# bernardo-torres/1d-spectral-optimal-transport

Hardware: AMD Instinct MI355X
Metric: sot_loss_evals_per_sec (higher is better)
Workload: dtype f32

## Files before the change

1d-spectral-optimal-transport_amd/csrc/sot_forward_full.inc:

```

#ifdef SOT_STAMPS
#define SOT_PH(sacc, i) do { if ((sacc) != nullptr) { __builtin_amdgcn_sched_barrier(0); const unsigned long long now_ = __builtin_readcyclecounter(); \
                              (sacc)[i] += now_ - (sacc)[15]; (sacc)[15] = now_; __builtin_amdgcn_sched_barrier(0); } } while (0)
#else
#define SOT_PH(sacc, i) do { } while (0)
#endif

template <int NSTEPS>
__device__ __forceinline__ float mass_column_nx(const float* part, int c)
{
    constexpr int NFULL = NSTEPS >> 4;
    constexpr int NREAD = NFULL + ((NSTEPS & 15) ? 1 : 0);
    float pre[NREAD];
#pragma unroll
    for (int h = 0; h < NREAD; ++h) pre[h] = part[(h << 5) + c];
    float a0 = 0.0f, a1 = 0.0f, a2 = 0.0f, a3 = 0.0f;
#pragma unroll
    for (int h = 0; h < NFULL; ++h) {
        a0 = pre[h];
        a1 += a0; a0 = 0.0f;
        if ((((h + 1) << 4) & (15 << 4)) == 0) {
            a2 += a1; a1 = 0.0f;
            if ((((h + 1) << 4) & (15 << 8)) == 0) { a3 += a2; a2 = 0.0f; }
        }
// ... 401 lines not shown
#pragma unroll
            for (int s2 = 0; s2 < CHUNK; ++s2) acc += v[s2];
            part[id] = acc;
        }
    }
    }
    SOT_PH(sacc, 3);
    if constexpr (!COLUMNS) row_sync<NW>();
    SOT_PH(sacc, 4);
    __builtin_amdgcn_s_setprio(kMassPrio);
    if (NW >= 2) {
        if (wv < 2 && !(wv == 1 && dn)) {
            const float* raw = wv ? V : U;
            float* cb = colbuf + 32 * wv;
            if (lane < 32) {
                if constexpr (RT) cb[lane] = mass_column<SQ>(raw, part + wv * NT, mp, lane);
                else cb[lane] = mass_column_nx<Geo::NSTEPS>(part + wv * NT, lane);
            }
            __builtin_amdgcn_fence(__ATOMIC_RELEASE, "wavefront");
            __builtin_amdgcn_wave_barrier();
            __builtin_amdgcn_fence(__ATOMIC_ACQUIRE, "wavefront");
            float S;
            if constexpr (RT) S = mass_fold<SQ>(raw, cb, mp.n);
            else S = mass_fold_nx<(SQ && !PRESQ), N, SWZ>(raw, cb);
            if (lane == 0) { Sv[wv] = S; Sv[2 + wv] = 1.0f / guard_mass(S); }
        }
    } else {
        const int half = lane >> 5, col = lane & 31;
        const bool use_y = half && !dn;
        float* cb = colbuf + 32 * half;
        if constexpr (RT) cb[col] = mass_column<SQ>(use_y ? V : U, part + (use_y ? NT : 0), mp, col);
        else cb[col] = mass_column_nx<Geo::NSTEPS>(part + (use_y ? NT : 0), col);
        __builtin_amdgcn_fence(__ATOMIC_RELEASE, "wavefront");
        __builtin_amdgcn_wave_barrier();
        __builtin_amdgcn_fence(__ATOMIC_ACQUIRE, "wavefront");
        float S;
        if constexpr (RT) S = mass_fold<SQ>(use_y ? V : U, cb, mp.n);
        else S = mass_fold_nx<(SQ && !PRESQ), N, SWZ>(use_y ? V : U, cb);
        if (col == 0) { Sv[half] = S; Sv[2 + half] = 1.0f / guard_mass(S); }
    }
    __builtin_amdgcn_s_setprio(0);
    const int e0 = t * CPT;
    const int h0 = e0 + 4 * ownf, h1 = e0 + 4 * (1 - ownf);
    if (x_ident) {
        if constexpr (CPT == 8) {
            const float4 v0 = *reinterpret_cast<const float4*>(U + h0), v1 = *reinterpret_cast<const float4*>(U + h1);
            wx[0] = v0.x; wx[1] = v0.y; wx[2] = v0.z; wx[3] = v0.w; wx[4] = v1.x; wx[5] = v1.y; wx[6] = v1.z; wx[7] = v1.w;
        } else {
#pragma unroll
            for (int k = 0; k < CPT; ++k) wx[k] = U[e0 + k];
        }
    } else if (psx != nullptr) {
#pragma unroll
        for (int k = 0; k < CPT; ++k) wx[k] = U[psx[k]];
    } else {
#pragma unroll
        for (int k = 0; k < CPT; ++k) {
            const int sx = (e0 + k < (RT ? a.n : N)) ? a.xperm[e0 + k] : N + 1;
            wx[k] = U[SWZ ? (sx ^ (((sx >> 5) & 1) << 2)) : sx];
        }
    }
    if (y_ident) {
        if constexpr (CPT == 8) {
            const float4 v0 = *reinterpret_cast<const float4*>(V + h0), v1 = *reinterpret_cast<const float4*>(V + h1);
            wy[0] = v0.x; wy[1] = v0.y; wy[2] = v0.z; wy[3] = v0.w; wy[4] = v1.x; wy[5] = v1.y; wy[6] = v1.z; wy[7] = v1.w;
        } else {
#pragma unroll
            for (int k = 0; k < CPT; ++k) wy[k] = V[e0 + k];
        }
    } else if (psy != nullptr) {
#pragma unroll
        for (int k = 0; k < CPT; ++k) wy[k] = V[psy[k]];
    } else {
#pragma unroll
        for (int k = 0; k < CPT; ++k) {
            const int sy = (e0 + k < (RT ? a.n : N)) ? a.yperm[e0 + k] : N + 1;
            wy[k] = V[SWZ ? (sy ^ (((sy >> 5) & 1) << 2)) : sy];
        }
    }
    if ((N < Geo::CAP || RT) && e0 + CPT > (RT ? a.n : N)) {
#pragma unroll
        for (int k = 0; k < CPT; ++k) {
            if (e0 + k >= (RT ? a.n : N)) { wx[k] = 0.0f; wy[k] = 0.0f; }
        }
    }
    SOT_PH(sacc, 5);
    row_sync<NW>();
    SOT_PH(sacc, 6);

    Sx = Sv[0]; Sy = dn ? Sx : Sv[1];
    const float rSx = Sv[2], rSy = dn ? rSx : Sv[3];
    const float Sxh = guard_mass(Sx), Syh = guard_mass(Sy);
    double px[CPT], py[CPT];
    double runx = 0.0, runy = 0.0;
    {
        float qx[CPT], qy[CPT];
        uint32_t risk = 0xFFFFFFFFu;
#pragma unroll
        for (int k = 0; k < CPT; ++k) {
            qx[k] = div_by_row_constant((SQ && !PRESQ) ? wx[k] * wx[k] : wx[k], Sxh, rSx, risk);
            qy[k] = div_by_row_constant((SQ && !PRESQ) ? wy[k] * wy[k] : wy[k], Syh, rSy, risk);
        }
        const bool slow = (risk < kFastDivMinBits) || !(Sxh <= 0x1p40f) || !(Syh <= 0x1p40f);
        if (__builtin_amdgcn_ballot_w64(slow) != 0ull) {
            asm volatile("; IEEE division fallback" ::: "memory");
#pragma unroll
            for (int k = 0; k < CPT; ++k) {
                qx[k] = ((SQ && !PRESQ) ? wx[k] * wx[k] : wx[k]) / Sxh;
                qy[k] = ((SQ && !PRESQ) ? wy[k] * wy[k] : wy[k]) / Syh;
            }
        }
#pragma unroll
        for (int k = 0; k < CPT; ++k) {
            runx += (double)qx[k]; runy += (double)qy[k];
            px[k] = runx; py[k] = runy;
        }
    }
    const double inx = wave_incl_scan(runx), iny = wave_incl_scan(runy);
    double exx = wave_shift_right1(inx), exy = wave_shift_right1(iny);
    if (NW > 1 && lane == kWave - 1) { wtot[wv] = inx; wtot[NW + wv] = iny; }
    SOT_PH(sacc, 7);
    row_sync<NW>();
    SOT_PH(sacc, 8);
    if constexpr (NW > 1) {
        double ox = 0.0, oy = 0.0;
        for (int w = 0; w < wv; ++w) { ox += wtot[w]; oy += wtot[NW + w]; }
        exx += ox; exy += oy;
    }
#pragma unroll
    for (int k = 0; k < CPT; ++k) { cu[k] = (float)(exx + px[k]); cv[k] = (float)(exy + py[k]); }
    if constexpr (TO_LDS) {
        if (CPT % 4 == 0 && (N == Geo::CAP || e0 + CPT <= N)) {
#pragma unroll
            for (int k = 0; k + 3 < CPT; k += 4) {
                *reinterpret_cast<float4*>(U + e0 + k) = make_float4(cu[k], cu[k + 1], cu[k + 2], cu[k + 3]);
                *reinterpret_cast<float4*>(V + e0 + k) = make_float4(cv[k], cv[k + 1], cv[k + 2], cv[k + 3]);
            }
        } else {
#pragma unroll
            for (int k = 0; k < CPT; ++k) {
                if (e0 + k < N) { U[e0 + k] = cu[k]; V[e0 + k] = cv[k]; }
            }
        }
    }
    if (nxt_x != nullptr) fetch_row<G, CPT, NX>(nxt_x, nxt_y, t, a.n, rx, ry);
    if constexpr (TO_LDS) row_sync<NW>();
}

template <int G, int CPT, int ROWS, int NX>
__device__ __forceinline__ void owner_perm_slots(const FwdArgs& a, const int* perm, int t, int (&ps)[CPT])
{
    using Geo = FullGeo<G, CPT, ROWS, false, NX>;
    constexpr int N = Geo::N;
    const int nreal = Geo::RT ? a.n : N;
#pragma unroll
    for (int k = 0; k < CPT; ++k) {
        const int sx = (t * CPT + k < nreal) ? perm[t * CPT + k] : N + 1;
        ps[k] = Geo::SWZ ? (sx ^ (((sx >> 5) & 1) << 2)) : sx;
    }
}

constexpr int kFwdMinWaves = 1;
constexpr int kRt512MinWaves = 4;

template <int G, int CPT, int ROWS, int GRAD, int NX>
__device__ __forceinline__ void rowpos_row_setup(const FwdArgs& a, const FullCtx& c, int64_t rowc, int (&ix)[CPT], int (&iy)[CPT], int (&psx)[CPT], int (&psy)[CPT])
{
    using Geo = FullGeo<G, CPT, ROWS, GRAD, NX>;
    constexpr int N = Geo::N, NW = Geo::NW, PAD = Geo::PAD;
    static_assert(ROWS == 1 && NX == 0 && CPT == 8, "per-row positions: one row per workgroup, rows that fill the 8-element geometry");
    const int t = c.t;
    const uint16_t* const pr = a.perm_in + rowc * (2 * (int64_t)N);
    const float* const xp = a.xpos + rowc * a.xps;
    const float* const yp = a.ypos + rowc * a.yps;
    const uint4 qx = *reinterpret_cast<const uint4*>(pr + t * CPT), qy = *reinterpret_cast<const uint4*>(pr + N + t * CPT);
    float vx[CPT], vy[CPT];
#pragma unroll
    for (int k = 0; k < CPT; ++k) { vx[k] = xp[t + k * G]; vy[k] = yp[t + k * G]; }
    const uint32_t wqx[4] = {qx.x, qx.y, qx.z, qx.w}, wqy[4] = {qy.x, qy.y, qy.z, qy.w};
#pragma unroll
    for (int k = 0; k < CPT; ++k) {
        ix[k] = (int)((wqx[k >> 1] >> (16 * (k & 1))) & (uint32_t)(N - 1));
        iy[k] = (int)((wqy[k >> 1] >> (16 * (k & 1))) & (uint32_t)(N - 1));
        psx[k] = Geo::SWZ ? (ix[k] ^ (((ix[k] >> 5) & 1) << 2)) : ix[k];
        psy[k] = Geo::SWZ ? (iy[k] ^ (((iy[k] >> 5) & 1) << 2)) : iy[k];
    }
    float* const Um = c.U; float* const Vm = c.V;
#pragma unroll
    for (int k = 0; k < CPT; ++k) { Um[t + k * G] = vx[k]; Vm[t + k * G] = vy[k]; }
    row_sync<NW>();
    float gx[CPT], gy[CPT];
#pragma unroll
    for (int k = 0; k < CPT; ++k) { gx[k] = Um[ix[k]]; gy[k] = Vm[iy[k]]; }
    float* const PXw = const_cast<float*>(c.PX); float* const PYw = const_cast<float*>(c.PY);
    *reinterpret_cast<float4*>(PXw + t * CPT) = make_float4(gx[0], gx[1], gx[2], gx[3]);
    *reinterpret_cast<float4*>(PXw + t * CPT + 4) = make_float4(gx[4], gx[5], gx[6], gx[7]);
    *reinterpret_cast<float4*>(PYw + t * CPT) = make_float4(gy[0], gy[1], gy[2], gy[3]);
    *reinterpret_cast<float4*>(PYw + t * CPT + 4) = make_float4(gy[4], gy[5], gy[6], gy[7]);
    if (t < PAD) PXw[t - PAD] = gx[0];
    if (t == G - 1) { PXw[N] = gx[CPT - 1]; PYw[N] = gy[CPT - 1]; }
    row_sync<NW>();
}

template <int G, int CPT, int ROWS, int PM, bool LIM, bool SQ, int NX = 0, bool RP = false>
__global__ __launch_bounds__(ROWS * G, (G == 512 && NX < 0) ? kRt512MinWaves : (CPT == 17) ? kFwd17MinWaves : kFwdMinWaves) void sot_forward_full_kernel(const FwdArgs a)
{
    static_assert(!RP || (ROWS == 1 && NX == 0 && CPT == 8), "per-row positions: one row per workgroup, rows that fill the 8-element geometry");
    using Geo = FullGeo<G, CPT, ROWS, false, NX>;
    constexpr FullLayout L = Geo::L;
    constexpr int N = Geo::N, NW = Geo::NW, E = Geo::E, GA = Geo::GA, PAD = Geo::PAD;
    extern __shared__ __attribute__((aligned(16))) float smem[];
    const int64_t row_step = (int64_t)gridDim.x * ROWS;
    int64_t row0 = (int64_t)blockIdx.x * ROWS;
    float rx[CPT], ry[CPT];
    FullCtx cm = full_setup<G, CPT, ROWS, false, NX, RP>(a, smem);
    if constexpr (RP) { cm.x_ident = false; cm.y_ident = false; }
    const FullCtx c = cm;
    if constexpr (NW == 1) __syncthreads();
    const int rg = c.rg, t = c.t, lane = c.lane, wv = c.wv;
    float* const V = c.V; float* const red = c.red;
    const float* const Uw = c.Uw;
    if (row0 < a.B) {
        const int64_t r = min(row0 + rg, a.B - 1);
        fetch_row<G, CPT, NX>(a.x + r * a.xs, a.y + r * a.ys, t, a.n, rx, ry);
    }

#ifdef SOT_STAMPS
    unsigned long long sbuf[16] = {};
    unsigned long long* const sacc = (threadIdx.x == 0 && blockIdx.x == gridDim.x / 2) ? sbuf : nullptr;
#else
    constexpr unsigned long long* sacc = nullptr;
#endif
    constexpr bool HOIST_PERM = CPT <= 9;
    int psx[HOIST_PERM ? CPT : 1] = {}, psy[HOIST_PERM ? CPT : 1] = {};
    if constexpr (HOIST_PERM && !RP) {
        if (!c.x_ident) owner_perm_slots<G, CPT, ROWS, NX>(a, a.xperm, t, psx);
        if (!c.y_ident) owner_perm_slots<G, CPT, ROWS, NX>(a, a.yperm, t, psy);
    }
    for (; row0 < a.B; row0 += row_step) {
        const int64_t row = row0 + rg;
        const bool valid = row < a.B;
        const bool more = row0 + row_step < a.B;
        const int64_t rn = min(row0 + row_step + rg, a.B - 1);
        float wx[CPT], wy[CPT], cu[CPT], cv[CPT];
        float Sx, Sy;
#ifdef SOT_STAMPS
        if (sacc != nullptr) sacc[15] = __builtin_readcyclecounter();
#endif
        if constexpr (RP) {
            int ix[CPT], iy[CPT];
            rowpos_row_setup<G, CPT, ROWS, false, NX>(a, c, min(row, a.B - 1), ix, iy, psx, psy);
        }
        full_build_cdfs<G, CPT, ROWS, false, SQ, NX>(a, c, rx, ry, more ? a.x + rn * a.xs : nullptr,
                                                     more ? a.y + rn * a.ys : nullptr, wx, wy, Sx, Sy, cu, cv, sacc, HOIST_PERM ? psx : nullptr,
                                                     HOIST_PERM ? psy : nullptr);
        SOT_PH(sacc, 9);

        float acc = 0.0f;
        __builtin_amdgcn_s_setprio(kWalkPrio);
        if (GA == G || t < GA) {
            constexpr int VOFF = L.nU - L.padcap + PAD;
            const int D0 = t * E;
            (void)VOFF;
            const uint32_t ub1 = lds_addr(Uw) - 4u;
            const uint32_t vd1 = lds_addr(V) + 4u * (uint32_t)D0 + ub1;
            const uint32_t pb = merge_path_fixed32<N + PAD, N>(ub1, vd1, D0);
            SOT_PH(sacc, 10);
            const uint32_t ou = pb + 4u;
            const uint32_t ov = vd1 - pb;
            constexpr uint32_t ROWB = 4u * (uint32_t)L.rowf;
            if (ROWS == 1 || rg == ROWS - 1) acc = merge_walk_full<E, PM, LIM, ROWB>(ou, ov, D0 == 0, a.p);
            else if (ROWS == 2 || rg == ROWS - 2) acc = merge_walk_full<E, PM, LIM, 2u * ROWB>(ou, ov, D0 == 0, a.p);
            else if (ROWS == 3 || rg == ROWS - 3) acc = merge_walk_full<E, PM, LIM, 3u * ROWB>(ou, ov, D0 == 0, a.p);
            else acc = merge_walk_full<E, PM, LIM, 4u * ROWB>(ou, ov, D0 == 0, a.p);
        }
        __builtin_amdgcn_s_setprio(0);
        SOT_PH(sacc, 11);
        acc = wave_sum(acc);
        if (NW == 1) {
            if (lane == 0 && valid && a.row_loss) store_row_loss(a.row_loss, row, acc, a.mt.counters != nullptr);
            row_sync<NW>();
        } else {
            if (lane == 0) red[wv] = acc;
            row_sync<NW>();
            if (t == 0 && valid && a.row_loss) {
                float tot = red[0];
#pragma unroll
                for (int w = 1; w < NW; ++w) tot += red[w];
                store_row_loss(a.row_loss, row, tot, a.mt.counters != nullptr);
            }
        }
        SOT_PH(sacc, 12);
#ifdef SOT_STAMPS
        if (sacc != nullptr) sacc[0] += 1;
#endif
    }
#ifdef SOT_STAMPS
    if (sacc != nullptr) { for (int i = 0; i < 16; ++i) g_stamps[i] = sacc[i]; }
#endif
    if (a.mt.counters != nullptr) batch_mean_tail<ROWS * G>(a.mt, a.row_loss, a.B, reinterpret_cast<double*>(smem));
}


constexpr int kAreaMinWaves = 1;
template <int G, int CPT, int ROWS, bool SQ, int NX = 0>
__global__ __launch_bounds__(ROWS * G, (CPT == 17) ? kFwd17MinWaves : kAreaMinWaves) void sot_area_full_kernel(const FwdArgs a)
{
    using Geo = FullGeo<G, CPT, ROWS, false, NX>;
    constexpr FullLayout L = Geo::L;
    constexpr int N = Geo::N, NW = Geo::NW;
    extern __shared__ __attribute__((aligned(16))) float smem[];
    const int64_t row_step = (int64_t)gridDim.x * ROWS;
    int64_t row0 = (int64_t)blockIdx.x * ROWS;
    const int tid = threadIdx.x;
    FullCtx c;
    c.rg = __builtin_amdgcn_readfirstlane(tid / G);
    c.t = tid - c.rg * G;
    c.lane = tid & (kWave - 1);
    c.wv = __builtin_amdgcn_readfirstlane(c.t >> 6);
    const int rg = c.rg, t = c.t, lane = c.lane, wv = c.wv;
    float rx[CPT], ry[CPT];
    if (row0 < a.B) {
        const int64_t r = min(row0 + rg, a.B - 1);
        fetch_row<G, CPT, NX>(a.x + r * a.xs, a.y + r * a.ys, t, a.n, rx, ry);
    }
    c.dn = a.flags & SOT_FLAG_DONT_NORMALIZE;
    float* const base = smem + rg * L.rowf;
    c.U = base + L.padcap; c.V = base + L.nU; c.part = base + L.part; c.colbuf = base + L.colbuf;
    c.wtot = reinterpret_cast<double*>(base + L.wtot);
    c.red = base + L.red; c.Sv = c.red + NW;
    c.Uw = c.U; c.PX = nullptr; c.PY = nullptr;
    c.x_ident = true; c.y_ident = true;
    if (a.ident != nullptr) { c.x_ident = a.ident[0] != 0; c.y_ident = a.ident[1] != 0; }
    float dx[CPT];
    {
        const int e0 = t * CPT;
        float pe[CPT + 1];
        const int nreal = Geo::RT ? a.n : N;
#pragma unroll
        for (int k = 0; k <= CPT; ++k) pe[k] = a.xpos[min(e0 + k, nreal - 1)];
#pragma unroll
        for (int k = 0; k < CPT; ++k) dx[k] = (e0 + k + 1 < nreal) ? pe[k + 1] - pe[k] : 0.0f;
    }
    float* const red = c.red;
#ifdef SOT_STAMPS
    unsigned long long sbuf[16] = {};
    unsigned long long* const sacc = (threadIdx.x == 0 && blockIdx.x == gridDim.x / 2) ? sbuf : nullptr;
#endif

    for (; row0 < a.B; row0 += row_step) {
        const int64_t row = row0 + rg;
        const bool valid = row < a.B;
        const bool more = row0 + row_step < a.B;
        const int64_t rn = min(row0 + row_step + rg, a.B - 1);
        float wx[CPT], wy[CPT], cu[CPT], cv[CPT];
        float Sx, Sy;
#ifdef SOT_STAMPS
        if (sacc != nullptr) sacc[15] = __builtin_readcyclecounter();
        full_build_cdfs<G, CPT, ROWS, false, SQ, NX, false>(a, c, rx, ry, more ? a.x + rn * a.xs : nullptr,
                                                            more ? a.y + rn * a.ys : nullptr, wx, wy, Sx, Sy, cu, cv, sacc);
        SOT_PH(sacc, 9);
#else
        full_build_cdfs<G, CPT, ROWS, false, SQ, NX, false>(a, c, rx, ry, more ? a.x + rn * a.xs : nullptr,
                                                            more ? a.y + rn * a.ys : nullptr, wx, wy, Sx, Sy, cu, cv);
#endif
        float acc = 0.0f;
#pragma unroll
        for (int k = 0; k < CPT; ++k) acc = fmaf(fabsf(cu[k] - cv[k]), dx[k], acc);
        acc = wave_sum(acc);
        if (NW == 1) {
            if (lane == 0 && valid && a.row_loss) store_row_loss(a.row_loss, row, acc, a.mt.counters != nullptr);
            row_sync<NW>();
        } else {
            if (lane == 0) red[wv] = acc;
            row_sync<NW>();
            if (t == 0 && valid && a.row_loss) {
                float tot = red[0];
#pragma unroll
                for (int w = 1; w < NW; ++w) tot += red[w];
                store_row_loss(a.row_loss, row, tot, a.mt.counters != nullptr);
            }
        }
#ifdef SOT_STAMPS
        SOT_PH(sacc, 10);
        if (sacc != nullptr) sacc[0] += 1;
#endif
    }
#ifdef SOT_STAMPS
    if (sacc != nullptr) { for (int i = 0; i < 16; ++i) g_stamps[i] = sacc[i]; }
#endif
    if (a.mt.counters != nullptr) batch_mean_tail<ROWS * G>(a.mt, a.row_loss, a.B, reinterpret_cast<double*>(smem));
}

__device__ __forceinline__ double half_incl_scan(double v)
{
    v += dpp_f64_shr<kRowShr1>(v);
    v += dpp_f64_shr<kRowShr2>(v);
    v += dpp_f64_shr<kRowShr4>(v);
    v += dpp_f64_shr<kRowShr8>(v);
    v += dpp_f64<kRowBcast15, 0xA>(v);
    return v;
}
__device__ __forceinline__ double half_shift_right1(double v, int l)
{
    const double s = dpp_f64<kWaveShr1>(v);
    return l == 0 ? 0.0 : s;
}
__device__ __forceinline__ float half_sum(float v, int h)
{
    v += dpp_f32<kRowShr1>(v);
    v += dpp_f32<kRowShr2>(v);
    v += dpp_f32<kRowShr4>(v);
    v += dpp_f32<kRowShr8>(v);
    v += dpp_f32<kRowBcast15, 0xA>(v);
    const float t0 = __int_as_float(__builtin_amdgcn_readlane(__float_as_int(v), 31));
    const float t1 = __int_as_float(__builtin_amdgcn_readlane(__float_as_int(v), 63));
    return h ? t1 : t0;
}

template <int CPT, int N>
__device__ __forceinline__ void half_fetch(const float* __restrict__ x, const float* __restrict__ y, int l, float (&rx)[CPT], float (&ry)[CPT])
{
    constexpr int NK = (N + 31) >> 5;
#pragma unroll
    for (int k = 0; k < CPT; ++k) {
        rx[k] = 0.0f; ry[k] = 0.0f;
        if (k < NK) {
            const int e = l + 32 * k;
            if ((k + 1) * 32 <= N || e < N) { rx[k] = x[e]; ry[k] = y[e]; }
        }
    }
}

template <int CPT, bool SQ, int N>
__device__ __forceinline__ void half_stage(float* U, float* V, float* colbuf, int l, const float (&rx)[CPT], const float (&ry)[CPT])
{
    constexpr int NSTEPS = N >> 5, NK = (N + 31) >> 5;
    float ax = 0.0f, ay = 0.0f;
#pragma unroll
    for (int k = 0; k < NK; ++k) {
        const int e = l + 32 * k;
        if ((k + 1) * 32 <= N || e < N) { U[e] = rx[k]; V[e] = ry[k]; }
        if (k < NSTEPS) { ax += SQ ? rx[k] * rx[k] : rx[k]; ay += SQ ? ry[k] * ry[k] : ry[k]; }
    }
    colbuf[l] = ax; colbuf[32 + l] = ay;
}

template <int CPT, bool SQ, int N>
__device__ __forceinline__ void half_cdfs(const FwdArgs& a, const float* U, const float* V, const float* colbuf, int l, bool dn, bool x_ident,
                                          bool y_ident, float (&cu)[CPT], float (&cv)[CPT])
{
    const int e0 = l * CPT;
    const float Sx = mass_fold_nx<SQ, N, false>(U, colbuf);
    const float Sy = dn ? Sx : mass_fold_nx<SQ, N, false>(V, colbuf + 32);
    float wx[CPT], wy[CPT];
#pragma unroll
    for (int k = 0; k < CPT; ++k) {
        const bool in = e0 + k < N;
        const int sx = in ? (x_ident ? e0 + k : a.xperm[e0 + k]) : 0;
        const int sy = in ? (y_ident ? e0 + k : a.yperm[e0 + k]) : 0;
        wx[k] = in ? U[sx] : 0.0f;
        wy[k] = in ? V[sy] : 0.0f;
    }
    const float Sxh = guard_mass(Sx), Syh = guard_mass(Sy);
    const float rSx = 1.0f / Sxh, rSy = 1.0f / Syh;
    double px[CPT], py[CPT];
    double runx = 0.0, runy = 0.0;
    {
        float qx[CPT], qy[CPT];
        uint32_t risk = 0xFFFFFFFFu;
#pragma unroll
        for (int k = 0; k < CPT; ++k) {
            qx[k] = div_by_row_constant(SQ ? wx[k] * wx[k] : wx[k], Sxh, rSx, risk);
            qy[k] = div_by_row_constant(SQ ? wy[k] * wy[k] : wy[k], Syh, rSy, risk);
        }
        const bool slow = (risk < kFastDivMinBits) || !(Sxh <= 0x1p40f) || !(Syh <= 0x1p40f);
        if (__builtin_amdgcn_ballot_w64(slow) != 0ull) {
#pragma unroll
            for (int k = 0; k < CPT; ++k) {
                qx[k] = (SQ ? wx[k] * wx[k] : wx[k]) / Sxh;
                qy[k] = (SQ ? wy[k] * wy[k] : wy[k]) / Syh;
            }
        }
#pragma unroll
        for (int k = 0; k < CPT; ++k) {
            runx += (double)qx[k]; runy += (double)qy[k];
            px[k] = runx; py[k] = runy;
        }
    }
    const double exx = half_shift_right1(half_incl_scan(runx), l), exy = half_shift_right1(half_incl_scan(runy), l);
#pragma unroll
    for (int k = 0; k < CPT; ++k) { cu[k] = (float)(exx + px[k]); cv[k] = (float)(exy + py[k]); }
}

template <int CPT, int ROWS, bool SQ, int N>
__global__ __launch_bounds__(ROWS * 32) void sot_area_half_kernel(const FwdArgs a)
{
    constexpr int CAP = 32 * CPT, NSTEPS = N >> 5, NK = (N + 31) >> 5;
    static_assert(ROWS % 2 == 0 && NK <= CPT && N <= CAP && NSTEPS >= 1 && NSTEPS < 16, "two half-wave rows per wave; one partial ATen chunk per column");
    static_assert((N >> 3) == NSTEPS * 4, "no left-over 8-lane vectors (N mod 32 < 8)");
    constexpr int ROWF = 2 * (CAP + 4) + 64 + 8;
    extern __shared__ __attribute__((aligned(16))) float smem[];
    const int tid = threadIdx.x, lane = tid & (kWave - 1), l = lane & 31, h = lane >> 5, rs = tid >> 5;
    float* const U = smem + rs * ROWF;
    float* const V = U + CAP + 4;
    float* const colbuf = V + CAP + 4;
    const bool dn = a.flags & SOT_FLAG_DONT_NORMALIZE;
    bool x_ident = true, y_ident = true;
    if (a.ident != nullptr) { x_ident = a.ident[0] != 0; y_ident = a.ident[1] != 0; }
    const int64_t row_step = (int64_t)gridDim.x * ROWS;
    int64_t row0 = (int64_t)blockIdx.x * ROWS;
    const int e0 = l * CPT;
    float dx[CPT];
    {
        float pe[CPT + 1];
#pragma unroll
        for (int k = 0; k <= CPT; ++k) pe[k] = a.xpos[min(e0 + k, N - 1)];
#pragma unroll
        for (int k = 0; k < CPT; ++k) dx[k] = (e0 + k + 1 < N) ? pe[k + 1] - pe[k] : 0.0f;
    }
    float rx[CPT], ry[CPT];
    if (row0 < a.B) { const int64_t r = min(row0 + rs, a.B - 1); half_fetch<CPT, N>(a.x + r * a.xs, a.y + r * a.ys, l, rx, ry); }

    for (; row0 < a.B; row0 += row_step) {
        const int64_t row = row0 + rs;
        const bool valid = row < a.B;
        half_stage<CPT, SQ, N>(U, V, colbuf, l, rx, ry);
        if (row0 + row_step < a.B) { const int64_t r = min(row0 + row_step + rs, a.B - 1); half_fetch<CPT, N>(a.x + r * a.xs, a.y + r * a.ys, l, rx, ry); }
        row_sync<1>();
        float cu[CPT], cv[CPT];
        half_cdfs<CPT, SQ, N>(a, U, V, colbuf, l, dn, x_ident, y_ident, cu, cv);
        float acc = 0.0f;
#pragma unroll
        for (int k = 0; k < CPT; ++k) acc = fmaf(fabsf(cu[k] - cv[k]), dx[k], acc);
        acc = half_sum(acc, h);
        if (l == 0 && valid && a.row_loss) store_row_loss(a.row_loss, row, acc, a.mt.counters != nullptr);
        row_sync<1>();
    }
    if (a.mt.counters != nullptr) batch_mean_tail<ROWS * 32>(a.mt, a.row_loss, a.B, reinterpret_cast<double*>(smem));
}

template <int CPT, int ROWS, int PM, bool LIM, bool SQ, int N>
struct HalfRowGeo {
    static constexpr int CAP = 32 * CPT, K = 2 * N, E = merge_steps(K, 32), GA = (K + E - 1) / E, PAD = GA * E - K;
    static constexpr int PADCAP = align4(E) + 4, NU = PADCAP + CAP + 4, NV = CAP + 4;
    static constexpr int POFF = NU + NV + 64;
    static constexpr int ROWF = POFF + NU + NV;
    static_assert(GA <= 32 && PAD + 1 <= PADCAP, "every lane walks at most one segment; room for the virtual predecessor");
};

template <int CPT, int ROWS, int PM, bool LIM, bool SQ, int N>
__global__ __launch_bounds__(ROWS * 32) void sot_forward_half_kernel(const FwdArgs a)
{
    using H = HalfRowGeo<CPT, ROWS, PM, LIM, SQ, N>;
    constexpr int CAP = H::CAP, NSTEPS = N >> 5, NK = (N + 31) >> 5, E = H::E, GA = H::GA, PAD = H::PAD;
    static_assert(ROWS % 2 == 0 && NK <= CPT && N <= CAP && NSTEPS >= 1 && NSTEPS < 16 && (N >> 3) == NSTEPS * 4, "see sot_area_half_kernel");
    extern __shared__ __attribute__((aligned(16))) float smem[];
    const int tid = threadIdx.x, lane = tid & (kWave - 1), l = lane & 31, h = lane >> 5, rs = tid >> 5;
    float* const base = smem + rs * H::ROWF;
    float* const U = base + H::PADCAP;
    float* const V = base + H::NU;
    float* const colbuf = base + H::NU + H::NV;
    float* const PX = U + H::POFF;
    float* const PY = V + H::POFF;
    const bool dn = a.flags & SOT_FLAG_DONT_NORMALIZE;
    bool x_ident = true, y_ident = true;
    if (a.ident != nullptr) { x_ident = a.ident[0] != 0; y_ident = a.ident[1] != 0; }
    for (int e = l; e < N; e += 32) { PX[e] = a.xpos[e]; PY[e] = a.ypos[e]; }
    if (l < PAD) { PX[l - PAD] = a.xpos[0]; U[l - PAD] = 0.0f; }
    if (l == 0) {
        PX[N] = a.xpos[N - 1]; PY[N] = a.ypos[N - 1];
        U[N] = INFINITY; V[N] = INFINITY;
        U[-PAD - 1] = -INFINITY; V[-1] = -INFINITY;
    }
    const int64_t row_step = (int64_t)gridDim.x * ROWS;
    int64_t row0 = (int64_t)blockIdx.x * ROWS;
    const int e0 = l * CPT;
    float rx[CPT], ry[CPT];
    if (row0 < a.B) { const int64_t r = min(row0 + rs, a.B - 1); half_fetch<CPT, N>(a.x + r * a.xs, a.y + r * a.ys, l, rx, ry); }
    row_sync<1>();

    for (; row0 < a.B; row0 += row_step) {
        const int64_t row = row0 + rs;
        const bool valid = row < a.B;
        half_stage<CPT, SQ, N>(U, V, colbuf, l, rx, ry);
        row_sync<1>();
        float cu[CPT], cv[CPT];
        half_cdfs<CPT, SQ, N>(a, U, V, colbuf, l, dn, x_ident, y_ident, cu, cv);
        row_sync<1>();
#pragma unroll
        for (int k = 0; k < CPT; ++k) {
            if (e0 + k < N) { U[e0 + k] = cu[k]; V[e0 + k] = cv[k]; }
        }
        if (row0 + row_step < a.B) { const int64_t r = min(row0 + row_step + rs, a.B - 1); half_fetch<CPT, N>(a.x + r * a.xs, a.y + r * a.ys, l, rx, ry); }
        row_sync<1>();
        float acc = 0.0f;
        if (GA == 32 || l < GA) {
            const int D0 = l * E;
            const uint32_t ub1 = lds_addr(U - PAD) - 4u;
            const uint32_t vd1 = lds_addr(V) + 4u * (uint32_t)D0 + ub1;
            const uint32_t pb = merge_path_fixed32<N + PAD, N>(ub1, vd1, D0);
            acc = merge_walk_full<E, PM, LIM, 4u * (uint32_t)H::POFF>(pb + 4u, vd1 - pb, D0 == 0, a.p);
        }
        acc = half_sum(acc, h);
        if (l == 0 && valid && a.row_loss) store_row_loss(a.row_loss, row, acc, a.mt.counters != nullptr);
        row_sync<1>();
    }
    if (a.mt.counters != nullptr) batch_mean_tail<ROWS * 32>(a.mt, a.row_loss, a.B, reinterpret_cast<double*>(smem));
}

#if SOT_FULL_FWD || SOT_FULL_RT_FWD
template <int G, int CPT, int ROWS, bool SQ, int NX>
static hipError_t launch_area_full(const FwdArgs& a, hipStream_t s)
{
    auto kern = sot_area_full_kernel<G, CPT, ROWS, SQ, NX>;
    constexpr FullLayout L = full_layout<G, CPT, ROWS, false, NX>();
    const size_t lds = sizeof(float) * (size_t)ROWS * (size_t)L.rowf;
    constexpr int block = ROWS * G;
    static GridCache cache;
    const int grid_cap = cached_resident_grid(cache, kern, block, lds);
    const int64_t want = (a.B + ROWS - 1) / ROWS;
    const int grid = persistent_grid(want, grid_cap);
    (void)hipGetLastError();
    launch_maybe_profiled(kern, grid, block, lds, s, a);
    return hipGetLastError();
}

template <int G, int CPT, int ROWS, int NX = 0>
static hipError_t dispatch_area_full_g(const FwdArgs& a, hipStream_t s)
{
    return (a.flags & SOT_FLAG_SQUARE) ? launch_area_full<G, CPT, ROWS, true, NX>(a, s) : launch_area_full<G, CPT, ROWS, false, NX>(a, s);
}


template <int CPT, int ROWS, int N>
static hipError_t dispatch_area_half(const FwdArgs& a, hipStream_t s)
{
    constexpr size_t lds = sizeof(float) * (size_t)ROWS * (2 * (32 * CPT + 4) + 64 + 8);
    constexpr int block = ROWS * 32;
    const int64_t want = (a.B + ROWS - 1) / ROWS;
    (void)hipGetLastError();
    if (a.flags & SOT_FLAG_SQUARE) {
        auto kern = sot_area_half_kernel<CPT, ROWS, true, N>;
        static GridCache cache;
        launch_maybe_profiled(kern, persistent_grid(want, cached_resident_grid(cache, kern, block, lds)), block, lds, s, a);
    } else {
        auto kern = sot_area_half_kernel<CPT, ROWS, false, N>;
        static GridCache cache;
        launch_maybe_profiled(kern, persistent_grid(want, cached_resident_grid(cache, kern, block, lds)), block, lds, s, a);
    }
    return hipGetLastError();
}
#endif
#if SOT_FULL_FWD
hipError_t dispatch_area_full(const FwdArgs& a, hipStream_t s)
{
    switch (a.n) {
        case 512: return dispatch_area_full_g<64, 8, 4>(a, s);
        case 1024: return dispatch_area_full_g<128, 8, 2>(a, s);
        case 2048: return dispatch_area_full_g<256, 8, 1>(a, s);
        case 4096: return dispatch_area_full_g<512, 8, 1>(a, s);
        case 8192: return dispatch_area_full_g<1024, 8, 1>(a, s);
        case 129:
            return dispatch_area_half<5, 8, 129>(a, s);
        case 2049: return dispatch_area_full_g<256, 9, 1, 2049>(a, s);
        case 257:
            return dispatch_area_full_g<64, 5, 4, 257>(a, s);
        case 513: return dispatch_area_full_g<64, 9, 4, 513>(a, s);
        case 1025:
            return dispatch_area_full_g<64, 17, 4, 1025>(a, s);
        default: return hipErrorInvalidConfiguration;
    }
}

#endif

__device__ __forceinline__ void store_grad16(float* dst, float a, float b, float c, float d)
{
    *reinterpret_cast<float4*>(dst) = make_float4(a, b, c, d);
}

__device__ __forceinline__ void lds_store(uint32_t addr, float v)
{
    *reinterpret_cast<__attribute__((address_space(3))) float*>((uintptr_t)addr) = v;
}

constexpr int kGradStagedMinBins = 1025;
template <int G, int N>
__device__ __forceinline__ void flush_row_grad(const float* lds_row, float* grow, int t)
{
    const int sh = (int)((reinterpret_cast<uintptr_t>(grow) >> 2) & 3u);
    float* const A = grow - sh;
    const int nch = (sh + N + 3) >> 2;
    const float4* const src = reinterpret_cast<const float4*>(lds_row);
    constexpr int NCH_MAX = (N + 3 + 3) >> 2;
#pragma unroll
    for (int i = 0; i < (NCH_MAX + G - 1) / G; ++i) {
        const int cidx = t + i * G;
        if (cidx < nch) {
            const float4 v = src[cidx];
            const int lo = 4 * cidx;
            if (lo >= sh && lo + 4 <= sh + N) {
                *reinterpret_cast<float4*>(A + lo) = v;
            } else {
                if (lo + 0 >= sh && lo + 0 < sh + N) A[lo + 0] = v.x;
                if (lo + 1 >= sh && lo + 1 < sh + N) A[lo + 1] = v.y;
                if (lo + 2 >= sh && lo + 2 < sh + N) A[lo + 2] = v.z;
                if (lo + 3 >= sh && lo + 3 < sh + N) A[lo + 3] = v.w;
            }
        }
    }
}

template <int G, int CPT, int ROWS, int PM, bool LIM, bool SQ, int NX = 0, bool WANT_X = true, bool SLIM = false, int MINB = 1, bool RP = false>
__global__ __launch_bounds__(ROWS * G, MINB) void sot_backward_full_kernel(const BwdArgs b)
{
    static_assert(!RP || (ROWS == 1 && NX == 0 && CPT == 8), "per-row positions (see sot_forward_full_kernel): one row per workgroup, rows that fill the 8-element geometry");
    static_assert(!(SLIM && WANT_X), "SLIM is a y-only layout");
    constexpr int GR = SLIM ? 2 : 1;
    using Geo = FullGeo<G, CPT, ROWS, GR, NX>;
    constexpr FullLayout L = Geo::L;
    constexpr int N = Geo::N, NW = Geo::NW, E = Geo::E, GA = Geo::GA, PAD = Geo::PAD;
    constexpr bool WITH_LOSS = !WANT_X;
    extern __shared__ __attribute__((aligned(16))) float smem[];
    const FwdArgs& a = b.f;
    const int64_t row_step = (int64_t)gridDim.x * ROWS;
    int64_t row0 = (int64_t)blockIdx.x * ROWS;
    float rx[CPT], ry[CPT];
    FullCtx cm = full_setup<G, CPT, ROWS, GR, NX, RP>(a, smem);
    if constexpr (RP) { cm.x_ident = false; cm.y_ident = false; }
    const FullCtx c = cm;
    if constexpr (NW == 1) __syncthreads();
    const int rg = c.rg, t = c.t, lane = c.lane, wv = c.wv;
    float* const U = c.U; float* const V = c.V;
    const float* const Uw = c.Uw;
    const float* const GU = U + L.goff; const float* const GV = V + L.goff;
    double* const wtot = c.wtot;
    if (row0 < a.B) {
        const int64_t r = min(row0 + rg, a.B - 1);
        fetch_row<G, CPT, NX>(a.x + r * a.xs, a.y + r * a.ys, t, a.n, rx, ry);
    }

#ifdef SOT_STAMPS
    unsigned long long sbuf[16] = {};
    unsigned long long* const sacc = (threadIdx.x == 0 && blockIdx.x == gridDim.x / 2) ? sbuf : nullptr;
#else
    constexpr unsigned long long* sacc = nullptr;
#endif

    constexpr bool STAGE_OUT = NX >= kGradStagedMinBins;
    const bool stage_x = STAGE_OUT && WANT_X && b.gx != nullptr && c.x_ident;
    const bool stage_y = STAGE_OUT && b.gy != nullptr && c.y_ident;
    int64_t pend_row = -1;
    (void)stage_x; (void)stage_y;

    for (; row0 < a.B; row0 += row_step) {
        const int64_t row = row0 + rg;
        const bool valid = row < a.B;
        const int64_t rowc = valid ? row : a.B - 1;
        const bool more = row0 + row_step < a.B;
        const int64_t rn = min(row0 + row_step + rg, a.B - 1);
        float wx[CPT], wy[CPT], cu[CPT], cv[CPT];
        float Sx, Sy;
#ifdef SOT_STAMPS
        if (sacc != nullptr) sacc[15] = __builtin_readcyclecounter();
#endif
        if constexpr (STAGE_OUT) {
            if (pend_row >= 0) {
                if constexpr (WANT_X) { if (stage_x) flush_row_grad<G, N>(GU, b.gx + pend_row * (int64_t)N, t); }
                if (stage_y) flush_row_grad<G, N>(GV, b.gy + pend_row * (int64_t)N, t);
            }
            pend_row = valid ? row : -1;
        }
        int ix[RP ? CPT : 1] = {}, iy[RP ? CPT : 1] = {}, psx[RP ? CPT : 1] = {}, psy[RP ? CPT : 1] = {};
        if constexpr (RP) rowpos_row_setup<G, CPT, ROWS, GR, NX>(a, c, rowc, ix, iy, psx, psy);
        full_build_cdfs<G, CPT, ROWS, GR, SQ, NX>(a, c, rx, ry, more ? a.x + rn * a.xs : nullptr,
                                                  more ? a.y + rn * a.ys : nullptr, wx, wy, Sx, Sy, cu, cv, sacc, RP ? psx : nullptr, RP ? psy : nullptr);
        SOT_PH(sacc, 9);

        __builtin_amdgcn_s_setprio(kWalkPrio);
        float lacc = 0.0f, lq = 0.0f;
        if (GA == G || t < GA) {
            const uint32_t poff4 = 4u * (uint32_t)((ROWS - rg) * L.rowf);
            constexpr uint32_t GOFF4 = 4u * (uint32_t)L.goff;
            bool slot = !SLIM;
            const int D0 = t * E;
            const uint32_t uw32 = lds_addr(Uw);
            const uint32_t ub1 = uw32 - 4u;
            const uint32_t vd1 = lds_addr(V) + 4u * (uint32_t)D0 + ub1;
            const uint32_t pb = merge_path_fixed32<N + PAD, N>(ub1, vd1, D0);
            const uint32_t ou = pb + 4u, ov = vd1 - pb;
            float qprev = fmaxf(lds_load(pb), lds_load(ov - 4u));
            float ua = lds_load(ou), vb = lds_load(ov), xa = lds_load(ou + poff4), yb = lds_load(ov + poff4);
            float dcur = 0.0f;
            lq = (D0 == 0) ? 0.0f : qprev;
            if (D0 == 0) {
                qprev = __int_as_float(0x7fc00000);
            } else if (fminf(ua, vb) == qprev) {
                const float q0 = qprev;
                const float cst = transport_cost<PM>(c.PX[lower_rank(U, N, q0)], c.PY[lower_rank(V, N, q0)], a.p);
                dcur = (LIM && q0 > 1.0f) ? 0.0f : cst;
            }
            uint32_t pu = ou, pv = ov;
            uint32_t prev = uw32 + 4u * (uint32_t)(PAD + N);
#pragma unroll SOT_FULL_WALK_UNROLL
            for (int s2 = 0; s2 < E; ++s2) {
                const bool tu = ua <= vb;
                const float q = tu ? ua : vb;
                float cst = transport_cost<PM>(xa, yb, a.p);
                if constexpr (WITH_LOSS) {
                    float delta = q - lq;
                    if (LIM && q > 1.0f) delta = 0.0f;
                    lacc = fmaf(delta, cst, lacc);
                    lq = q;
                }
                if (LIM && q > 1.0f) cst = 0.0f;
                const bool new_run = !(q == qprev);
                if (!SLIM || slot) lds_store(prev + GOFF4, new_run ? (dcur - cst) : 0.0f);
                dcur = new_run ? cst : dcur;
                qprev = q;
                prev = tu ? pu : pv;
                if constexpr (SLIM) slot = !tu;
                const uint32_t nx = prev + 4u;
                pu = tu ? nx : pu;
                pv = tu ? pv : nx;
                const float nv = lds_load(nx);
                const float np = lds_load(nx + poff4);
                ua = tu ? nv : ua;
                xa = tu ? np : xa;
                vb = tu ? vb : nv;
                yb = tu ? yb : np;
            }
            {
                const float qn = fminf(ua, vb);
                float cn = transport_cost<PM>(xa, yb, a.p);
                if ((LIM && qn > 1.0f) || (t == GA - 1)) cn = 0.0f;
                const bool new_run = !(qn == qprev) || (t == GA - 1);
                if (!SLIM || slot) lds_store(prev + GOFF4, new_run ? (dcur - cn) : 0.0f);
            }
        }
        __builtin_amdgcn_s_setprio(0);
        SOT_PH(sacc, 10);
        if constexpr (WITH_LOSS) {
            lacc = wave_sum(lacc);
            if (lane == 0) c.red[wv] = lacc;
        }
        row_sync<NW>();
        SOT_PH(sacc, 11);
        if constexpr (WITH_LOSS) {
            if (t == 0 && valid && a.row_loss) {
                float tot = c.red[0];
#pragma unroll
                for (int w = 1; w < NW; ++w) tot += c.red[w];
                store_row_loss(a.row_loss, row, tot, a.mt.counters != nullptr);
            }
        }

        const int e0 = t * CPT;
        double ga[CPT], gb[CPT];
        double runx = 0.0, runy = 0.0;
        {
            float gu[CPT], gv[CPT];
            if constexpr (CPT % 4 == 0) {
#pragma unroll
                for (int k = 0; k + 3 < CPT; k += 4) {
                    float4 u4 = make_float4(0.0f, 0.0f, 0.0f, 0.0f);
                    if constexpr (WANT_X) u4 = *reinterpret_cast<const float4*>(GU + e0 + k);
                    const float4 v4 = *reinterpret_cast<const float4*>(GV + e0 + k);
                    gu[k] = u4.x; gu[k + 1] = u4.y; gu[k + 2] = u4.z; gu[k + 3] = u4.w;
                    gv[k] = v4.x; gv[k + 1] = v4.y; gv[k + 2] = v4.z; gv[k + 3] = v4.w;
                }
            } else {
#pragma unroll
                for (int k = 0; k < CPT; ++k) { gu[k] = WANT_X ? GU[e0 + k] : 0.0f; gv[k] = GV[e0 + k]; }
            }
            if (N < Geo::CAP && e0 + CPT > N) {
#pragma unroll
                for (int k = 0; k < CPT; ++k) {
                    if (e0 + k >= N) { gu[k] = 0.0f; gv[k] = 0.0f; }
                }
            }
#pragma unroll
            for (int k = CPT - 1; k >= 0; --k) {
                if constexpr (WANT_X) runx += (double)gu[k];
                runy += (double)gv[k];
                ga[k] = runx;
                gb[k] = runy;
            }
        }
        const double pinx = WANT_X ? wave_incl_scan(runx) : 0.0, piny = wave_incl_scan(runy);
        const double totwx = WANT_X ? wave_last(pinx) : 0.0, totwy = wave_last(piny);
        double exx = totwx - pinx, exy = totwy - piny;
        if (NW > 1) {
            if (lane == 0) { if constexpr (WANT_X) wtot[wv] = totwx; wtot[NW + wv] = totwy; }
            row_sync<NW>();
            double ox = 0.0, oy = 0.0;
            for (int w = NW - 1; w > wv; --w) { if constexpr (WANT_X) ox += wtot[w]; oy += wtot[NW + w]; }
            exx += ox;
            exy += oy;
        }
        SOT_PH(sacc, 12);
        const bool need_dots = WANT_X || !c.dn;
        double dotx = 0.0, doty = 0.0;
#pragma unroll
        for (int k = 0; k < CPT; ++k) {
            gb[k] += exy;
            if constexpr (WANT_X) ga[k] += exx;
        }
        double totx = 0.0, toty = 0.0;
        if (need_dots) {
#pragma unroll
            for (int k = 0; k < CPT; ++k) {
                const float sy = SQ ? wy[k] * wy[k] : wy[k];
                doty += gb[k] * (double)sy;
                if constexpr (WANT_X) {
                    const float sx = SQ ? wx[k] * wx[k] : wx[k];
                    dotx += ga[k] * (double)sx;
                }
            }
            if constexpr (WANT_X) dotx = wave_sum(dotx);
// ... 620 lines not shown
```

Baseline: 251.3 million.

## Add double-buffered LDS ring with async global-to-LDS loads for area kernel

For the G=256, CPT=8, single-row area configuration, adds a dedicated persistent-row path that streams x/y rows straight into a two-slot LDS ring using global_load_lds. Each row is prefetched two rounds ahead, and the next row's chunk sums, mass fold and owner reads are overlapped with the current row's scan and loss computation. The goal is to hide global memory latency and cut per-row barrier stalls. In exchange it brings a new LDS layout, manual vmcnt waits and more code complexity, and it only applies to that one configuration.

```diff
diff --git a/1d-spectral-optimal-transport_amd/csrc/sot_forward_full.inc b/1d-spectral-optimal-transport_amd/csrc/sot_forward_full.inc
--- a/1d-spectral-optimal-transport_amd/csrc/sot_forward_full.inc
+++ b/1d-spectral-optimal-transport_amd/csrc/sot_forward_full.inc
@@ -727,10 +727,276 @@
 }
 
 
+struct AreaRingLayout {
+    int slot;
+    int part, colbuf, wtot, red;
+    int rowf;
+};
+template <int G>
+__host__ __device__ constexpr AreaRingLayout area_ring_layout()
+{
+    constexpr int N = 8 * G, NW = G / kWave, NT = 32 * ((N >> 5) >> 4);
+    AreaRingLayout L{};
+    L.slot = 2 * N;
+    L.part = 2 * L.slot;
+    L.colbuf = L.part + 2 * NT;
+    L.wtot = L.colbuf + 64;
+    L.red = L.wtot + 4 * NW;
+    L.rowf = align4(L.red + NW + 4);
+    return L;
+}
+
+template <int G, int CPT, int ROWS, int NX>
+__host__ __device__ constexpr bool area_uses_ring() { return NX == 0 && CPT == 8 && G == 256 && ROWS == 1; }
+template <int G, int CPT, int ROWS, int NX>
+__host__ __device__ constexpr size_t area_lds_bytes()
+{
+    if constexpr (area_uses_ring<G, CPT, ROWS, NX>()) return sizeof(float) * (size_t)ROWS * (size_t)area_ring_layout<G>().rowf;
+    else return sizeof(float) * (size_t)ROWS * (size_t)full_layout<G, CPT, ROWS, false, NX>().rowf;
+}
+
+typedef __attribute__((address_space(3))) void lds_void;
+constexpr int kRingPieces = 4;
+#define SOT_WAIT_VMCNT(n) __builtin_amdgcn_s_waitcnt(0x0F70 | (n))
+
+__device__ __forceinline__ void ring_barrier()
+{
+    asm volatile("s_waitcnt lgkmcnt(0)" ::: "memory");
+    __builtin_amdgcn_s_barrier();
+    asm volatile("" ::: "memory");
+}
+
+template <int G, int AUX>
+__device__ __forceinline__ void ring_request_row(const float* __restrict__ xrow, const float* __restrict__ yrow, float* slot, int wv, int lane)
+{
+    constexpr int N = 8 * G, PPA = N / 256;
+    static_assert(2 * PPA == kRingPieces * (G / kWave), "four pieces per wave");
+#pragma unroll
+    for (int j = 0; j < kRingPieces; ++j) {
+        const int pid = wv * kRingPieces + j;
+        const bool isy = pid >= PPA;
+        const int piece = isy ? pid - PPA : pid;
+        const int q = piece * 64 + lane;
+        const int qs = q ^ ((q >> 3) & 1);
+        __builtin_amdgcn_global_load_lds((isy ? yrow : xrow) + 4 * qs, (lds_void*)(slot + (isy ? N : 0) + piece * 256), 16, 0, AUX);
+    }
+}
+
+template <int G, bool SQ>
+__device__ __forceinline__ void ring_chunk_sums(const float* raw, float* part, int t, bool dn)
+{
+    constexpr int N = 8 * G, NT = G / 2;
+    const bool isy = t >= NT;
+    if (!(isy && dn)) {
+        const int task = isy ? t - NT : t;
+        const float* const src = raw + (isy ? N : 0) + ((task >> 5) << 9) + (task & 31);
+        const float* const srco = raw + (isy ? N : 0) + ((task >> 5) << 9) + ((task & 31) ^ 4);
+        float v[16];
+#pragma unroll
+        for (int k = 0; k < 16; ++k) { const float w = ((k & 1) ? srco : src)[k << 5]; v[k] = SQ ? w * w : w; }
+        float acc = 0.0f;
+#pragma unroll
+        for (int k = 0; k < 16; ++k) acc += v[k];
+        part[t] = acc;
+    }
+}
+
+template <int G>
+__device__ __forceinline__ void ring_fold(const float* part, float* colbuf, float* Sv, int wv, int lane, bool dn)
+{
+    constexpr int N = 8 * G, NT = G / 2;
+    __builtin_amdgcn_s_setprio(kMassPrio);
+    if (wv < 2 && !(wv == 1 && dn)) {
+        float* cb = colbuf + 32 * wv;
+        if (lane < 32) cb[lane] = mass_column_nx<(N >> 5)>(part + wv * NT, lane);
+        __builtin_amdgcn_fence(__ATOMIC_RELEASE, "wavefront");
+        __builtin_amdgcn_wave_barrier();
+        __builtin_amdgcn_fence(__ATOMIC_ACQUIRE, "wavefront");
+        float fin = 0.0f;
+#pragma unroll
+        for (int j = 0; j < 8; ++j) fin += ((cb[j] + cb[8 + j]) + cb[16 + j]) + cb[24 + j];
+        const float S = fin;
+        if (lane == 0) { Sv[wv] = S; Sv[2 + wv] = 1.0f / guard_mass(S); }
+    }
+    __builtin_amdgcn_s_setprio(0);
+}
+
+template <int G>
+__device__ __forceinline__ void ring_owner_reads(const FwdArgs& a, const float* raw, int t, bool x_ident, bool y_ident, float (&wx)[8], float (&wy)[8])
+{
+    constexpr int N = 8 * G;
+    const float* const U = raw; const float* const V = raw + N;
+    const int e0 = t * 8, ownf = (t >> 2) & 1;
+    const int h0 = e0 + 4 * ownf, h1 = e0 + 4 * (1 - ownf);
+    if (x_ident) {
+#pragma unroll
+        for (int k = 0; k < 4; ++k) { wx[k] = U[h0 + k]; wx[4 + k] = U[h1 + k]; }
+    } else {
+#pragma unroll
+        for (int k = 0; k < 8; ++k) wx[k] = U[staged_index(a.xperm[e0 + k], true)];
+    }
+    if (y_ident) {
+#pragma unroll
+        for (int k = 0; k < 4; ++k) { wy[k] = V[h0 + k]; wy[4 + k] = V[h1 + k]; }
+    } else {
+#pragma unroll
+        for (int k = 0; k < 8; ++k) wy[k] = V[staged_index(a.yperm[e0 + k], true)];
+    }
+}
+
+template <int G, int CPT, int ROWS, bool SQ>
+__device__ __forceinline__ void area_ring_rows(const FwdArgs& a)
+{
+    using Geo = FullGeo<G, CPT, ROWS, false, 0>;
+    constexpr AreaRingLayout L = area_ring_layout<G>();
+    constexpr int NW = Geo::NW;
+    constexpr int AUX = 2;
+    static_assert(CPT == 8 && Geo::SWZ && NW >= 2 && 2 * Geo::NT == G, "rows that fill their geometry on two or more waves");
+    static_assert(4 * sizeof(float) * ROWS * L.rowf <= 160 * 1024, "four workgroups per CU");
+    extern __shared__ __attribute__((aligned(16))) float smem[];
+    const int64_t row_step = (int64_t)gridDim.x * ROWS;
+    const int64_t row0 = (int64_t)blockIdx.x * ROWS;
+    const int tid = threadIdx.x;
+    const int rg = __builtin_amdgcn_readfirstlane(tid / G);
+    const int t = tid - rg * G;
+    const int lane = tid & (kWave - 1);
+    const int wv = __builtin_amdgcn_readfirstlane(t >> 6);
+    const bool dn = a.flags & SOT_FLAG_DONT_NORMALIZE;
+    float* const base = smem + rg * L.rowf;
+    float* const part = base + L.part; float* const colbuf = base + L.colbuf;
+    double* const wtot = reinterpret_cast<double*>(base + L.wtot);
+    float* const red = base + L.red; float* const Sv = red + NW;
+    bool x_ident = true, y_ident = true;
+    if (a.ident != nullptr) { x_ident = a.ident[0] != 0; y_ident = a.ident[1] != 0; }
+    float dx[CPT];
+    {
+        const int e0 = t * CPT;
+        float pe[CPT + 1];
+#pragma unroll
+        for (int k = 0; k <= CPT; ++k) pe[k] = a.xpos[min(e0 + k, Geo::N - 1)];
+#pragma unroll
+        for (int k = 0; k < CPT; ++k) dx[k] = (e0 + k + 1 < Geo::N) ? pe[k + 1] - pe[k] : 0.0f;
+    }
+#pragma unroll
+    for (int k = 0; k < CPT; ++k) asm volatile("" : "+v"(dx[k]) :: "memory");
+    const int rounds = (int)((a.B - row0 + row_step - 1) / row_step);
+    auto xrow = [&](int k) { return a.x + min(row0 + k * row_step + rg, a.B - 1) * a.xs; };
+    auto yrow = [&](int k) { return a.y + min(row0 + k * row_step + rg, a.B - 1) * a.ys; };
+#ifdef SOT_STAMPS
+    unsigned long long sbuf[16] = {};
+    unsigned long long* const sacc = (threadIdx.x == 0 && blockIdx.x == gridDim.x / 2) ? sbuf : nullptr;
+#endif
+
+    float wx[CPT], wy[CPT];
+    ring_request_row<G, AUX>(xrow(0), yrow(0), base, wv, lane);
+    if (rounds > 1) {
+        ring_request_row<G, AUX>(xrow(1), yrow(1), base + L.slot, wv, lane);
+        SOT_WAIT_VMCNT(kRingPieces);
+    } else {
+        SOT_WAIT_VMCNT(0);
+    }
+    ring_barrier();
+    ring_chunk_sums<G, SQ>(base, part, t, dn);
+    ring_barrier();
+    ring_fold<G>(part, colbuf, Sv, wv, lane, dn);
+    ring_owner_reads<G>(a, base, t, x_ident, y_ident, wx, wy);
+    SOT_WAIT_VMCNT(0);
+    ring_barrier();
+#ifdef SOT_STAMPS
+    if (sacc != nullptr) sacc[15] = __builtin_readcyclecounter();
+#endif
+
+    for (int k = 0; k < rounds; ++k) {
+        float* const cur = base + (k & 1) * L.slot;
+        const float* const nxt = base + ((k + 1) & 1) * L.slot;
+        if (k + 2 < rounds) ring_request_row<G, AUX>(xrow(k + 2), yrow(k + 2), cur, wv, lane);
+        if (k > 0 && t == 0) {
+            const int64_t rowp = row0 + (int64_t)(k - 1) * row_step + rg;
+            if (rowp < a.B && a.row_loss) {
+                float tot = red[0];
+#pragma unroll
+                for (int w = 1; w < NW; ++w) tot += red[w];
+                store_row_loss(a.row_loss, rowp, tot, a.mt.counters != nullptr);
+            }
+        }
+        if (k + 1 < rounds) ring_chunk_sums<G, SQ>(nxt, part, t, dn);
+        const float Sx = Sv[0], Sy = dn ? Sx : Sv[1];
+        const float rSx = Sv[2], rSy = dn ? rSx : Sv[3];
+        const float Sxh = guard_mass(Sx), Syh = guard_mass(Sy);
+        double px[CPT], py[CPT];
+        double runx = 0.0, runy = 0.0;
+        {
+            float qx[CPT], qy[CPT];
+            uint32_t risk = 0xFFFFFFFFu;
+#pragma unroll
+            for (int j = 0; j < CPT; ++j) {
+                qx[j] = div_by_row_constant(SQ ? wx[j] * wx[j] : wx[j], Sxh, rSx, risk);
+                qy[j] = div_by_row_constant(SQ ? wy[j] * wy[j] : wy[j], Syh, rSy, risk);
+            }
+            const bool slow = (risk < kFastDivMinBits) || !(Sxh <= 0x1p40f) || !(Syh <= 0x1p40f);
+            if (__builtin_amdgcn_ballot_w64(slow) != 0ull) {
+                asm volatile("; IEEE division fallback" ::: "memory");
+#pragma unroll
+                for (int j = 0; j < CPT; ++j) {
+                    qx[j] = (SQ ? wx[j] * wx[j] : wx[j]) / Sxh;
+                    qy[j] = (SQ ? wy[j] * wy[j] : wy[j]) / Syh;
+                }
+            }
+#pragma unroll
+            for (int j = 0; j < CPT; ++j) {
+                runx += (double)qx[j]; runy += (double)qy[j];
+                px[j] = runx; py[j] = runy;
+            }
+        }
+        const double inx = wave_incl_scan(runx), iny = wave_incl_scan(runy);
+        double exx = wave_shift_right1(inx), exy = wave_shift_right1(iny);
+        if (lane == kWave - 1) { wtot[wv] = inx; wtot[NW + wv] = iny; }
+        SOT_PH(sacc, 1);
+        ring_barrier();
+        SOT_PH(sacc, 2);
+        {
+            double ox = 0.0, oy = 0.0;
+            for (int w = 0; w < wv; ++w) { ox += wtot[w]; oy += wtot[NW + w]; }
+            exx += ox; exy += oy;
+        }
+        float acc = 0.0f;
+#pragma unroll
+        for (int j = 0; j < CPT; ++j) acc = fmaf(fabsf((float)(exx + px[j]) - (float)(exy + py[j])), dx[j], acc);
+        acc = wave_sum(acc);
+        if (lane == 0) red[wv] = acc;
+        if (k + 1 < rounds) {
+            ring_fold<G>(part, colbuf, Sv, wv, lane, dn);
+            ring_owner_reads<G>(a, nxt, t, x_ident, y_ident, wx, wy);
+        }
+        SOT_PH(sacc, 3);
+        SOT_WAIT_VMCNT(0);
+        SOT_PH(sacc, 4);
+        ring_barrier();
+        SOT_PH(sacc, 5);
+#ifdef SOT_STAMPS
+        if (sacc != nullptr) sacc[0] += 1;
+#endif
+    }
+    if (t == 0) {
+        const int64_t rowp = row0 + (int64_t)(rounds - 1) * row_step + rg;
+        if (rowp < a.B && a.row_loss) {
+            float tot = red[0];
+#pragma unroll
+            for (int w = 1; w < NW; ++w) tot += red[w];
+            store_row_loss(a.row_loss, rowp, tot, a.mt.counters != nullptr);
+        }
+    }
+#ifdef SOT_STAMPS
+    if (sacc != nullptr) { for (int i = 0; i < 16; ++i) g_stamps[i] = sacc[i]; }
+#endif
+    if (a.mt.counters != nullptr) batch_mean_tail<ROWS * G>(a.mt, a.row_loss, a.B, reinterpret_cast<double*>(smem));
+}
+
 constexpr int kAreaMinWaves = 1;
 template <int G, int CPT, int ROWS, bool SQ, int NX = 0>
 __global__ __launch_bounds__(ROWS * G, (CPT == 17) ? kFwd17MinWaves : kAreaMinWaves) void sot_area_full_kernel(const FwdArgs a)
 {
+    if constexpr (area_uses_ring<G, CPT, ROWS, NX>()) { area_ring_rows<G, CPT, ROWS, SQ>(a); return; }
     using Geo = FullGeo<G, CPT, ROWS, false, NX>;
     constexpr FullLayout L = Geo::L;
     constexpr int N = Geo::N, NW = Geo::NW;
@@ -1039,8 +1305,7 @@
 static hipError_t launch_area_full(const FwdArgs& a, hipStream_t s)
 {
     auto kern = sot_area_full_kernel<G, CPT, ROWS, SQ, NX>;
-    constexpr FullLayout L = full_layout<G, CPT, ROWS, false, NX>();
-    const size_t lds = sizeof(float) * (size_t)ROWS * (size_t)L.rowf;
+    constexpr size_t lds = area_lds_bytes<G, CPT, ROWS, NX>();
     constexpr int block = ROWS * G;
     static GridCache cache;
     const int grid_cap = cached_resident_grid(cache, kern, block, lds);
```

Result: faster. 253.9 million (median of 6 runs) (+1.0%).
